# ethz-asl/multipoint

Hardware: AMD Instinct MI355X
Metric: image-pairs/sec (detect+desc+match) @ 480x640 (higher is better)
Workload: dtype f32

## Files before the change

multipoint_amd/csrc/forward.hip:

```cpp
#include "host.h"

using namespace mp_host;

namespace {

int pick_mbw(int H, int W)
{
    long long best = -1;
    int arg = 32;
    for (int mbw : {32, 16, 8}) {
        const int tw = mbw, th = 256 / mbw;
        const long long area = (long long)((H + th - 1) / th) * th * ((W + tw - 1) / tw) * tw;
        if (best < 0 || area < best) { best = area; arg = mbw; }
    }
    return arg;
}

void prof_begin(mp_handle* h, const char* name, double flop, hipStream_t s)
{
    if (!h->prof) return;
    if (h->prof_used == h->prof_entries.size()) {
        ProfEntry e{};
        (void)hipEventCreate(&e.a); (void)hipEventCreate(&e.b);
        h->prof_entries.push_back(e);
// ... 215 lines not shown
    w.Lg = w.Q + px * 16 * el;
    w.X = w.Lg + npx * (f16 ? 128 : 80) * el;
    w.R = w.X + npx * 128 * el;
    w.lists = w.R + (f16 ? npx * 256 * el : 0);
    w.bytes = w.lists + 2 * 1024 * 4 + 256;
    return w;
}

struct ImageRoute {
    int counts[2] = {0, 0};
    std::vector<int> ids;
};

ImageRoute route_images(const mp_handle* h, const unsigned char* is_optical, int B)
{
    ImageRoute r;
    if (!h->cfg.multispectral) { r.counts[0] = B; return r; }
    r.ids.assign(1024, 0);
    for (int b = 0; b < B; ++b) {
        if (is_optical[b]) r.ids[512 + r.counts[1]++] = b;
        else r.ids[r.counts[0]++] = b;
    }
    return r;
}

template <typename T>
int run_forward(mp_handle* h, const float* images, const ImageRoute& route, int B, int H, int W, float* prob, float* logits, float* desc,
                hipStream_t s)
{
    constexpr bool f16 = std::is_same<T, _Float16>::value;
    const FwdWorkspace w = fwd_workspace(f16, B, H, W);
    int rc;
    if ((rc = ensure(h, h->fwd_ws, w.bytes))) return rc;
    if (f16 && (rc = ensure(h, h->f16_dummy, 4096))) return rc;
    char* ws = static_cast<char*>(h->fwd_ws.p);
    T *P = reinterpret_cast<T*>(ws + w.P), *Q = reinterpret_cast<T*>(ws + w.Q), *X = reinterpret_cast<T*>(ws + w.X);
    T *Lg = reinterpret_cast<T*>(ws + w.Lg), *R = reinterpret_cast<T*>(ws + w.R);
    int* lists = reinterpret_cast<int*>(ws + w.lists);
    if (h->prof_used > 4000) h->prof_used = 0;

    if (h->cfg.multispectral)
        MP_HIP(hipMemcpyAsync(lists, route.ids.data(), 1024 * 4, hipMemcpyHostToDevice, s));
    for (int e = 0; e < 2; ++e) {
        const int nb = route.counts[e];
        if (nb == 0) continue;
        const Encoder& E = h->enc[e];
        const int* list = h->cfg.multispectral ? lists + 512 * e : nullptr;
        const EncoderPlan plan = plan_encoder(h, E, nb, B, H, W);
        if (!plan.conv[0].fuse_first) run_first(h, E, plan.conv[0].in_planar == MP_LAYOUT_PLANAR, images, P, nb, H, W, list, s);
        int hh = E.first_pool ? H / 2 : H, ww = E.first_pool ? W / 2 : W;
        T* src = P;
        T* dst = Q;
        for (int i = 0; i < E.nconv; ++i) {
            const ConvLayer& L = E.conv[i];
            if ((rc = run_conv(h, L, plan.conv[i], src, L.cin, 0, i == E.nconv - 1 ? X : dst, L.cout, 0, nb, hh, ww, list, s,
                               &E.first, images))) return rc;
            if (L.pool) { hh /= 2; ww /= 2; }
            T* t = src; src = dst; dst = t;
        }
    }

    const int Hc = H / 8, Wc = W / 8, lstride = f16 ? 128 : 80;
    const long long npx = (long long)B * Hc * Wc;
    const int D = h->cfg.descriptor_size;
    const int hc = h->head_channels;
    const int headc = h->cfg.descriptor_head ? 2 * hc : hc;
    const int encc = h->heads3.cin;
    ConvLaunch c3, c1x1;
    if constexpr (f16) {
        c3.kernel = f16_kind(h, h->heads3, encc, 0, false);
        c1x1.kernel = Kernel::f16;
    } else {
        c3.kernel = wino43_kind(h, h->heads3, Hc, Wc, encc, 0, headc, 0);
        plan_split_vin(h, h->heads3, B, Hc, Wc, B, c3);
    }
    if ((rc = run_conv(h, h->heads3, c3, X, encc, 0, P, headc, 0, B, Hc, Wc, nullptr, s))) return rc;
    if (h->dbg.head_fuse && (!f16 || prob || logits || desc)) {
        typename std::conditional<f16, HeadTailParamsH, HeadTailParams>::type t{};
        t.x = P; t.xstride = headc; t.K = hc;
        if constexpr (f16) {
            t.wdet = h->det1.wpack_h; t.bdet = h->det1.bias_h; t.wdesc = h->desc1.wpack_h; t.bdesc = h->desc1.bias_h;
        } else {
            t.wdet = h->det1.wpack; t.bdet = h->det1.bias; t.wdesc = h->desc1.wpack; t.bdesc = h->desc1.bias;
        }
        t.sdet = h->det1.scale; t.tdet = h->det1.shift; t.sdesc = h->desc1.scale; t.tdesc = h->desc1.shift;
        t.D = D; t.npx = npx; t.B = B; t.Hc = Hc; t.Wc = Wc;
        t.prob = prob; t.logits_nchw = logits; t.desc = desc;
        t.softmax_mode = h->cfg.softmax_mode; t.normalize = h->cfg.normalize_descriptors ? 1 : 0; t.ncu = h->ncu;
        prof_begin(h, "heads.tail", 2.0 * hc * (65.0 + (desc ? D : 0)) * (double)npx, s);
        int miss;
        if constexpr (f16) miss = launch_head_tail_f16(t, s); else miss = launch_head_tail(t, s);
        prof_end(h, s);
        if (!miss) return launch_status(h);
        if (h->prof) --h->prof_used;
        if (!h->head_fallback_noted) {
            h->head_fallback_noted = true;
            fprintf(stderr, "[multipoint_hip] note: fused head tail not instantiated for %d head channels / descriptor size %d: "
                            "using the separate 1x1 convolution, softmax and normalisation launches\n", hc, D);
        }
    }
    if ((rc = run_conv(h, h->det1, c1x1, P, headc, 0, Lg, lstride, 0, B, Hc, Wc, nullptr, s))) return rc;
    if (prob || logits) {
        prof_begin(h, "det.softmax_shuffle", 0.0, s);
        if constexpr (f16) launch_det_post_f16(Lg, lstride, B, Hc, Wc, prob, logits, h->cfg.softmax_mode, s);
        else launch_det_post(Lg, lstride, B, Hc, Wc, prob, logits, h->cfg.softmax_mode, s);
        prof_end(h, s);
    }
    if (desc) {
        T* raw;
        if constexpr (f16) raw = R; else raw = desc;
        if ((rc = run_conv(h, h->desc1, c1x1, P, headc, hc, raw, D, 0, B, Hc, Wc, nullptr, s))) return rc;
        prof_begin(h, "desc.l2norm", 0.0, s);
        if constexpr (f16) launch_desc_l2norm_f16(R, desc, npx, D, h->cfg.normalize_descriptors ? 1 : 0, s);
        else if (h->cfg.normalize_descriptors) launch_desc_l2norm(desc, desc, npx, D, 1, s);
        prof_end(h, s);
    }
    return launch_status(h);
}


struct BsWorkspace { size_t A, Bf, X, G, part, ss, lists, bytes; };
BsWorkspace bs_workspace(int B, int H, int W, bool multispectral)
{
    const size_t px = (size_t)B * H * W, npx = px / 64;
    BsWorkspace w{};
    w.Bf = w.A + px * 64 * 4;
    w.X = w.Bf + px * 64 * 4;
    w.G = w.X + npx * 128 * 4;
    w.part = w.G + (multispectral ? px * 4 : 0);
    w.ss = w.part + (size_t)MP_BN_MAX_PARTS * 2 * 512 * 8;
    w.lists = w.ss + 1024 * 4;
    w.bytes = w.lists + 2 * 1024 * 4 + 256;
    return w;
}

struct BsContext {
    mp_handle* h;
    double* part;
    float *scale, *shift;
    float* stats;
    hipStream_t s;
};

void bs_stats(BsContext& c, const float* x, long long npx, int C)
{
    prof_begin(c.h, "bn.stats", 0.0, c.s);
    launch_bn_stats(x, npx, C, C, c.part, c.s);
    prof_end(c.h, c.s);
}

void bs_finalize(BsContext& c, const float* x, long long npx, int C, int c0, int nc, int layer)
{
    const BnLayer& L = c.h->bn_layers[layer];
    prof_begin(c.h, "bn.finalize", 0.0, c.s);
    launch_bn_finalize(c.part, npx, C, x, c0, nc, L.channels, L.gamma, L.beta, c.scale, c.shift,
                       c.stats ? c.stats + L.offset : nullptr, c.stats ? c.stats + L.offset + L.channels : nullptr, c.s);
    prof_end(c.h, c.s);
}

void bs_apply(BsContext& c, const float* x, float* y, int B, int H, int W, int C, bool relu, bool pool, const int* out_list)
{
    prof_begin(c.h, "bn.apply", 0.0, c.s);
    launch_bn_apply(x, y, B, H, W, C, c.scale, c.shift, relu, pool, out_list, c.s);
    prof_end(c.h, c.s);
}

// ... 190 lines not shown
```

multipoint_amd/csrc/head_tail.hip:

```cpp
#include "mp_common.h"
#include "mp_device.h"

#include <type_traits>

namespace {

__device__ __forceinline__ float acc_rd(float a)
{
    float x;
    asm volatile("v_accvgpr_read_b32 %0, %1" : "=v"(x) : "a"(a));
    return x;
}
template <int ND>
__global__ __launch_bounds__(256) void head_tail_kernel(const HeadTailParams p)
{
    constexpr int NT = 3 + ND;
    constexpr int NP = 96 + 32 * ND;
    constexpr int WCH = 4 * NT * 256;
    constexpr int XCH = 2 * 4 * 256;
    __shared__ __attribute__((aligned(16))) float wl[2 * WCH];
    __shared__ __attribute__((aligned(16))) float xl[2 * 4 * XCH];
    __shared__ __attribute__((aligned(16))) float prm[3 * NP];
    const int tid = threadIdx.x, lane = tid & 63;
    const int wave = __builtin_amdgcn_readfirstlane(tid >> 6);
    const int pl = lane & 31, hf = lane >> 5;
    for (int i = tid; i < NP; i += 256) {
        const bool det = i < 96;
        const int c = det ? i : i - 96;
        prm[i] = det ? p.bdet[c] : p.bdesc[c];
        prm[NP + i] = det ? p.sdet[c] : p.sdesc[c];
        prm[2 * NP + i] = det ? p.tdet[c] : p.tdesc[c];
    }

    const long long ntiles = (p.npx + 127) / 128;
    long long tile = blockIdx.x;
    long long px = 0;
    bool valid = false;
    unsigned xoff = 0, xoff_next = 0;
    const float *xbase = p.x, *xbase_next = p.x;
    auto place = [&](long long t, unsigned& off, const float*& base) __attribute__((always_inline)) {
        const long long q = (t * 4 + wave) * 32 + pl;
        off = (unsigned)(((q < p.npx ? q : p.npx - 1) - t * 128) * p.xstride + hf * 4) * 4u;
        base = p.x + t * 128 * p.xstride;
    };
    place(tile, xoff, xbase);
    const int nchunks = p.K >> 5;
    const unsigned wl_lds = (unsigned)(size_t)wl, xl_lds = (unsigned)(size_t)xl + (unsigned)wave * (XCH * 4u);

    auto chunk_dma = [&](int c, int buf, int j, bool next_tile) __attribute__((always_inline)) {
        if (j < NT) {
            const int nb = j < 3 ? j : j - 3;
            const float* w = j < 3 ? p.wdet : p.wdesc;
            const float* src = w + (((((long long)(nb >> 1) * nchunks + c) * 4 + wave) * 2 + (nb & 1)) * 64) * 4;
            lds_dma<4, 0, 0>(src, (unsigned)lane * 16u, wl_lds + (unsigned)(buf * WCH + (wave * NT + j) * 256) * 4u);
        } else {
            const int q = j - NT, part = q >> 2, g = q & 3;
            if (ND == 0 && part == 1) return;
            lds_dma<4, 0, 0>((next_tile ? xbase_next : xbase) + part * p.K + c * 32 + g * 8, next_tile ? xoff_next : xoff,
                             xl_lds + (unsigned)(buf * 4 * XCH + (part * 4 + g) * 256) * 4u);
        }
    };

#pragma unroll
    for (int j = 0; j < NT + 8; ++j) chunk_dma(0, 0, j, false);
    dma_wait();
    __syncthreads();

    for (;;) {
    const bool has_next = tile + gridDim.x < ntiles;
    if (has_next) place(tile + gridDim.x, xoff_next, xbase_next);
    px = (tile * 4 + wave) * 32 + pl;
    valid = px < p.npx;
    f32x16 acc[NT];
#pragma unroll
    for (int t = 0; t < NT; ++t)
#pragma unroll
        for (int r = 0; r < 16; ++r) acc[t][r] = 0.f;

    auto chunk = [&](int c, auto buf_tag, bool prefetch, bool next_tile) __attribute__((always_inline)) {
        constexpr int buf = decltype(buf_tag)::value;
        const float* const wb = wl + buf * WCH + lane * 4;
        const float* const xb = xl + wave * XCH + buf * 4 * XCH + lane * 4;
        f32x4 wf[2][NT], xd[2], xs[2];
        auto frags = [&](int slot, int g) __attribute__((always_inline)) {
#pragma unroll
            for (int t = 0; t < NT; ++t) wf[slot][t] = *reinterpret_cast<const f32x4*>(&wb[(g * NT + t) * 256]);
            xd[slot] = *reinterpret_cast<const f32x4*>(&xb[g * 256]);
            if (ND) xs[slot] = *reinterpret_cast<const f32x4*>(&xb[(4 + g) * 256]);
        };
        frags(0, 0);
#pragma unroll
        for (int g = 0; g < 4; ++g) {
            if (g + 1 < 4) frags((g + 1) & 1, g + 1);
#pragma unroll
            for (int e = 0; e < 4; ++e)
#pragma unroll
                for (int t = 0; t < NT; ++t) {
                    acc[t] = __builtin_amdgcn_mfma_f32_32x32x2f32(wf[g & 1][t][e], t < 3 ? xd[g & 1][e] : xs[g & 1][e], acc[t], 0, 0, 0);
                    __builtin_amdgcn_sched_barrier(0);
                    const int m = (g * 4 + e) * NT + t;
                    if (prefetch && m < NT + 8) chunk_dma(next_tile ? 0 : c + 1, buf ^ 1, m, next_tile);
                    __builtin_amdgcn_sched_barrier(0);
                }
        }
        dma_wait();
        __syncthreads();
    };
    using B0 = std::integral_constant<int, 0>;
    using B1 = std::integral_constant<int, 1>;
    for (int c = 0; c < nchunks; c += 2) {
        chunk(c, B0{}, true, false);
        const bool lastc = c + 2 >= nchunks;
        chunk(c + 1, B1{}, !lastc || has_next, lastc);
    }

    const int cell = (int)(px % ((long long)p.Hc * p.Wc));
    const int b = (int)(px / ((long long)p.Hc * p.Wc));
    const int hc = cell / p.Wc, wc = cell - hc * p.Wc;
    {
        float v[32];
#pragma unroll
        for (int t = 0; t < 2; ++t)
#pragma unroll
            for (int r = 0; r < 16; ++r) {
                const int c = 32 * t + (r & 3) + 8 * (r >> 2) + 4 * hf;
                v[16 * t + r] = (acc_rd(acc[t][r]) + prm[c]) * prm[NP + c] + prm[2 * NP + c];
            }
        float d = (acc_rd(acc[2][0]) + prm[64]) * prm[NP + 64] + prm[2 * NP + 64];
        d = __shfl(d, pl);
        if (p.logits_nchw && valid) {
            const long long plane = (long long)p.Hc * p.Wc;
            float* o = p.logits_nchw + (long long)b * 65 * plane + cell;
#pragma unroll
            for (int t = 0; t < 2; ++t)
#pragma unroll
                for (int r = 0; r < 16; ++r) o[(long long)(32 * t + (r & 3) + 8 * (r >> 2) + 4 * hf) * plane] = v[16 * t + r];
            if (hf == 0) o[64 * plane] = d;
        }
        if (p.prob) {
            float m = 0.f;
            if (p.softmax_mode == 0) {
                m = d;
#pragma unroll
                for (int i = 0; i < 32; ++i) m = fmaxf(m, v[i]);
                m = fmaxf(m, __shfl_xor(m, 32));
            }
            float s = 0.f;
#pragma unroll
            for (int i = 0; i < 32; ++i) { v[i] = __expf(v[i] - m); s += v[i]; }
            s += __shfl_xor(s, 32);
            s += __expf(d - m);
            if (p.softmax_mode == 1) s += 0.00001f;
            const float rs = 1.0f / s;
            if (valid) {
                const int H = p.Hc * 8, W = p.Wc * 8;
                float* o = p.prob + ((long long)b * H + hc * 8) * W + wc * 8 + 4 * hf;
#pragma unroll
                for (int t = 0; t < 2; ++t)
#pragma unroll
                    for (int q = 0; q < 4; ++q) {
                        const f32x4 o4 = {v[16 * t + 4 * q] * rs, v[16 * t + 4 * q + 1] * rs, v[16 * t + 4 * q + 2] * rs,
                                          v[16 * t + 4 * q + 3] * rs};
                        *reinterpret_cast<f32x4*>(o + (long long)(4 * t + q) * W) = o4;
                    }
            }
        }
    }
    if constexpr (ND > 0) {
        if (p.desc) {
            float ss = 0.f;
            f32x4 dv[ND * 4];
#pragma unroll
            for (int t = 0; t < ND; ++t)
#pragma unroll
                for (int q = 0; q < 4; ++q)
#pragma unroll
                    for (int e = 0; e < 4; ++e) {
                        const int c = 32 * t + 8 * q + 4 * hf + e;
                        const float x = (acc_rd(acc[3 + t][4 * q + e]) + prm[96 + c]) * prm[NP + 96 + c] + prm[2 * NP + 96 + c];
                        dv[4 * t + q][e] = x;
                        ss += x * x;
                    }
            if (p.normalize) {
                ss += __shfl_xor(ss, 32);
                const float rd = 1.0f / fmaxf(sqrtf(ss), 1e-12f);
#pragma unroll
                for (int i = 0; i < ND * 4; ++i) dv[i] = dv[i] * rd;
            }
            if (valid) {
                float* o = p.desc + px * (32 * ND) + 4 * hf;
#pragma unroll
                for (int t = 0; t < ND; ++t)
#pragma unroll
                    for (int q = 0; q < 4; ++q) *reinterpret_cast<f32x4*>(o + 32 * t + 8 * q) = dv[4 * t + q];
            }
        }
    }
    if (!has_next) return;
    tile += gridDim.x;
    xoff = xoff_next; xbase = xbase_next;
    }
}

}

int launch_head_tail(const HeadTailParams& p, hipStream_t s)
{
    if (p.K % 64 != 0 || p.npx <= 0) return 1;
    const int D = p.desc ? p.D : 0;
    const long long tiles = (p.npx + 127) / 128;
    const dim3 grid((unsigned)(tiles < p.ncu ? tiles : p.ncu)), block(256);
    switch (D) {
    case 0: hipLaunchKernelGGL(head_tail_kernel<0>, grid, block, 0, s, p); return 0;
    case 64: hipLaunchKernelGGL(head_tail_kernel<2>, grid, block, 0, s, p); return 0;
    case 128: hipLaunchKernelGGL(head_tail_kernel<4>, grid, block, 0, s, p); return 0;
    case 256: hipLaunchKernelGGL(head_tail_kernel<8>, grid, block, 0, s, p); return 0;
    default: return 1;
    }
}
```

multipoint_amd/csrc/host.h:

```cpp
#pragma once
#include "../../include/multipoint_hip.h"
#include "mp_common.h"

#include <cmath>
#include <cstdio>
#include <cstdlib>
#include <cstring>
#include <string>
#include <type_traits>
#include <vector>

namespace mp_host {

inline std::string g_create_error;

struct DevBuf {
    void* p = nullptr;
    size_t bytes = 0;
    DevBuf(void* p_ = nullptr, size_t bytes_ = 0) : p(p_), bytes(bytes_) {}
    DevBuf(DevBuf&& o) noexcept : p(o.p), bytes(o.bytes) { o.p = nullptr; o.bytes = 0; }
    ~DevBuf() { if (p) (void)hipFree(p); }
};

struct ConvLayer {
    const char* name = "";
    float *wpack = nullptr, *bias = nullptr, *scale = nullptr, *shift = nullptr;
    float* u43pack = nullptr;
    float *u43pack_f1 = nullptr, *bias_f1 = nullptr;
    _Float16* wpack_h = nullptr;
    float* bias_h = nullptr;
    int cin = 0, cout = 0, taps = 9, nslices = 0;
    bool pool = false, relu = true;
};

struct FirstLayer {
    int channels = 64;
    float *w = nullptr, *bias = nullptr, *scale = nullptr, *shift = nullptr;
    float *w_h = nullptr, *bias_h = nullptr;
    float *w_f1 = nullptr, *bias_f1 = nullptr;
};

struct Encoder {
    FirstLayer first;
    ConvLayer conv[7];
    int nconv = 7;
    bool first_pool = false;
};

struct BnLayer {
    std::string name;
    int channels = 0;
    float *gamma = nullptr, *beta = nullptr;
    long long offset = 0;
};

struct ProfEntry {
    const char* name;
    hipEvent_t a, b;
    double flop;
};

struct DebugSwitches {
    bool winograd = true, wino43 = true, fuse_first = true, fuse43 = true, head_fuse = true, vin = true, planar = true;
    bool xplanar = true, f16_res = true, f16_fuse1 = true;
    int wino43_gen = 0, persist = 8, splitk_max = 8, f16_res_groups = 3;
};

struct ConvPolicy {
    bool direct = false;
    bool wino43 = true;
    int wino43_gen = 0;
    int splitk_max = 8;
};

}

struct mp_handle {
    mp_handle(int device_, int ncu_, int xcd_shift_, const mp_host::DebugSwitches& dbg_)
        : device(device_), ncu(ncu_), xcd_shift(xcd_shift_), dbg(dbg_) {}
    const int device;
    const int ncu, xcd_shift;
    const mp_host::DebugSwitches dbg;
    std::string err;
    bool loaded = false;
    mp_model_config cfg{};
    mp_host::ConvPolicy policy;
    std::vector<mp_host::DevBuf> weights;
    mp_host::Encoder enc[2];
    mp_host::ConvLayer heads3, det1, desc1;
    mp_host::DevBuf fwd_ws;
    mp_host::DevBuf nms_ws;
    mp_host::DevBuf match_ws;
    mp_host::DevBuf metrics_ws;
    mp_host::DevBuf split_ws;
    mp_host::DevBuf vin_ws;
    mp_host::DevBuf bs_ws;
    std::vector<mp_host::BnLayer> bn_layers;
    float* bn_ident = nullptr;
    mp_host::DevBuf nms_state;
    mp_host::DevBuf kp_scratch;
    mp_host::DevBuf nms_total;
    int last_nms_rounds = 0;
    mp_host::DevBuf tie_state;
    float tie_eps = 6e-5f;
    int tie_min = 4;
    int tie_last_B = 0;
    mp_host::DevBuf tie_pairs;
    int tie_pairs_min = 16;
    int head_channels = 256;
    mp_host::DevBuf f16_dummy;
    int* pinned = nullptr;
    bool prof = false;
    bool head_fallback_noted = false;
    std::vector<mp_host::ProfEntry> prof_entries;
    size_t prof_used = 0;
};

namespace mp_host {

inline int fail(mp_handle* h, int code, const std::string& msg)
{
    if (h) h->err = msg; else g_create_error = msg;
    return code;
}

#define MP_HIP(expr)                                                                          \
    do {                                                                                      \
        hipError_t _e = (expr);                                                               \
        if (_e != hipSuccess)                                                                 \
            return fail(h, MP_EHIP, std::string(#expr) + ": " + hipGetErrorString(_e));       \
    } while (0)

inline int ensure(mp_handle* h, DevBuf& b, size_t bytes)
{
    if (b.bytes >= bytes) return MP_OK;
    if (b.p) { MP_HIP(hipFree(b.p)); b.p = nullptr; b.bytes = 0; }
    hipError_t e = hipMalloc(&b.p, bytes);
    if (e != hipSuccess) {
        b.p = nullptr;
        return fail(h, MP_ENOMEM, "hipMalloc(" + std::to_string(bytes) + " B): " + hipGetErrorString(e));
    }
    b.bytes = bytes;
    return MP_OK;
}

inline int ensure_zeroed(mp_handle* h, DevBuf& b, size_t bytes, hipStream_t s)
{
    if (b.bytes >= bytes) return MP_OK;
    const int rc = ensure(h, b, bytes);
    if (rc == MP_OK) MP_HIP(hipMemsetAsync(b.p, 0, bytes, s));
    return rc;
}

inline int launch_status(mp_handle* h)
{
    MP_HIP(hipGetLastError());
    return MP_OK;
}

}
```

multipoint_amd/csrc/model_load.hip:

```cpp
#include "host.h"

#include <map>
#include <numeric>

using namespace mp_host;

namespace {

template <typename T, typename D>
int upload(mp_handle* h, const std::vector<T>& v, D** out)
{
    static_assert(sizeof(T) == sizeof(D), "upload: element size");
    void* d = nullptr;
    MP_HIP(hipMalloc(&d, v.size() * sizeof(T)));
    h->weights.emplace_back(d, v.size() * sizeof(T));
    MP_HIP(hipMemcpy(d, v.data(), v.size() * sizeof(T), hipMemcpyHostToDevice));
    *out = static_cast<D*>(d);
    return MP_OK;
}

void free_weights(mp_handle* h)
{
    h->weights.clear();
    h->bn_layers.clear();
    h->bn_ident = nullptr;
    h->loaded = false;
}

uint16_t f2h_bits(float f)
{
    uint32_t x;
    std::memcpy(&x, &f, 4);
    const uint32_t sign = (x >> 16) & 0x8000u;
    x &= 0x7fffffffu;
    if (x >= 0x7f800000u) return (uint16_t)(sign | 0x7c00u | (x > 0x7f800000u ? 0x200u : 0u));
    if (x >= 0x477ff000u) return (uint16_t)(sign | 0x7c00u);
    if (x < 0x38800000u) {
        if (x < 0x33000000u) return (uint16_t)sign;
        const int e = (int)(x >> 23);
        const uint32_t m = (x & 0x7fffffu) | 0x800000u;
        const int shift = 126 - e;
        uint32_t r = m >> shift;
        const uint32_t rem = m & ((1u << shift) - 1u), halfway = 1u << (shift - 1);
        if (rem > halfway || (rem == halfway && (r & 1u))) ++r;
        return (uint16_t)(sign | r);
    }
    uint32_t r = (((x >> 23) - 112u) << 10) | ((x & 0x7fffffu) >> 13);
    const uint32_t rem = x & 0x1fffu;
    if (rem > 0x1000u || (rem == 0x1000u && (r & 1u))) ++r;
    return (uint16_t)(sign | r);
}

float h2f_bits(uint16_t h)
{
    const uint32_t sign = (uint32_t)(h & 0x8000u) << 16;
    const uint32_t e = (h >> 10) & 0x1fu, m = h & 0x3ffu;
    uint32_t x;
    if (e == 0) {
        if (m == 0) { x = sign; }
        else {
            int sh = 0;
            uint32_t mm = m;
            while (!(mm & 0x400u)) { mm <<= 1; ++sh; }
            x = sign | ((uint32_t)(113 - sh) << 23) | ((mm & 0x3ffu) << 13);
        }
    } else if (e == 31) {
        x = sign | 0x7f800000u | (m << 13);
    } else {
        x = sign | ((e + 112u) << 23) | (m << 13);
    }
    float f;
    std::memcpy(&f, &x, 4);
    return f;
}

float round_half(float f) { return h2f_bits(f2h_bits(f)); }

struct TensorMap {
    std::map<std::string, const mp_tensor*> m;
    std::map<std::string, bool> used;
    const float* get(const std::string& k, long long numel, std::string& err)
    {
        auto it = m.find(k);
        if (it == m.end()) { err = "missing key in state_dict: " + k; return nullptr; }
        if (it->second->numel != numel) {
            err = "size mismatch for " + k + ": got " + std::to_string(it->second->numel) +
                  " elements, expected " + std::to_string(numel);
            return nullptr;
        }
        used[k] = true;
        return it->second->data;
    }
};

bool bn_terms(TensorMap& tm, const std::string& prefix, int c, int padded, std::vector<float>& scale,
              std::vector<float>& shift, std::string& err)
{
    const float* g = tm.get(prefix + ".weight", c, err); if (!g) return false;
    const float* b = tm.get(prefix + ".bias", c, err); if (!b) return false;
    const float* m = tm.get(prefix + ".running_mean", c, err); if (!m) return false;
    const float* v = tm.get(prefix + ".running_var", c, err); if (!v) return false;
    if (tm.m.count(prefix + ".num_batches_tracked")) tm.used[prefix + ".num_batches_tracked"] = true;
    scale.assign(padded, 1.f); shift.assign(padded, 0.f);
    for (int i = 0; i < c; ++i) {
        const float invstd = 1.0f / std::sqrt(v[i] + 1e-5f);
        const float alpha = invstd * g[i];
        scale[i] = alpha;
        shift[i] = b[i] - m[i] * alpha;
// ... 212 lines not shown
                    for (int k = 0; k < 9; ++k) g += w2[((size_t)o * 64 + c) * 9 + k];
                    acc += g * t1[c];
                }
            b2f[o] = (float)acc;
        }
        std::vector<float> u4;
        pack_wino43_weights({w2}, {64}, 64, 64, u4, own ? nullptr : s1.data());
        if ((rc = upload(h, wf, &E.first.w_f1))) return rc;
        if ((rc = upload(h, bf, &E.first.bias_f1))) return rc;
        if ((rc = upload(h, u4, &E.conv[0].u43pack_f1))) return rc;
        if ((rc = upload(h, b2f, &E.conv[0].bias_f1))) return rc;
    }
    return MP_OK;
}

ConvPolicy conv_policy(const DebugSwitches& d, const mp_model_config& cfg)
{
    ConvPolicy p;
    p.direct = cfg.conv_algorithm == 3 || (cfg.conv_algorithm == 0 && !d.winograd);
    p.wino43 = !p.direct && (cfg.conv_algorithm != 0 || d.wino43);
    p.wino43_gen = cfg.conv_algorithm == 1 ? 0 : cfg.conv_algorithm == 2 ? 2 : d.wino43_gen;
    p.splitk_max = cfg.batch_invariant ? 1 : d.splitk_max;
    return p;
}

}

extern "C" {

int mp_load_weights(mp_handle* h, const mp_model_config* cfg, const mp_tensor* tensors, int n_tensors)
{
    if (!h) return MP_EINVAL;
    if (!cfg || (!tensors && n_tensors > 0)) return fail(h, MP_EINVAL, "mp_load_weights: NULL argument");
    if (cfg->channel_version < 0 || cfg->channel_version > 2)
        return fail(h, MP_EINVAL, "unsupported model config: channel_version must be 0, 1 or 2 (MultiPoint.py:38-53)");
    if (cfg->channel_version != 0 && cfg->key_layout == 1)
        return fail(h, MP_EINVAL, "unsupported model config: SuperPointMagicLeap has channel_version 0 shapes");
    if (!cfg->double_convolution && cfg->key_layout == 1)
        return fail(h, MP_EINVAL, "unsupported model config: SuperPointMagicLeap has two convolutions per stage");
    if (cfg->descriptor_head && cfg->descriptor_size != 64 && cfg->descriptor_size != 128 &&
        cfg->descriptor_size != 256)
        return fail(h, MP_EINVAL, "unsupported model config: descriptor_size must be 64, 128 or 256");
    if (cfg->conv_algorithm < 0 || cfg->conv_algorithm > 3)
        return fail(h, MP_EINVAL, "unsupported model config: conv_algorithm must be 0 (auto), 1 (winograd43), 2 (winograd43_general) or 3 (direct)");
    MP_HIP(hipSetDevice(h->device));
    free_weights(h);
    h->cfg = *cfg;
    h->policy = conv_policy(h->dbg, *cfg);
    TensorMap tm;
    for (int i = 0; i < n_tensors; ++i) {
        if (!tensors[i].name || (!tensors[i].data && tensors[i].numel > 0))
            return fail(h, MP_EINVAL, "mp_load_weights: tensor " + std::to_string(i) + " has NULL field");
        tm.m[tensors[i].name] = &tensors[i];
    }
    int rc;
    if (cfg->key_layout == 1 && (cfg->multispectral || cfg->batchnorm || cfg->final_batchnorm))
        return fail(h, MP_EINVAL, "unsupported model config: SuperPointMagicLeap key layout has one encoder and no BatchNorm");
    if (!cfg->batchnorm && cfg->key_layout == 0)
        return fail(h, MP_EINVAL, "unsupported model config: MultiPoint key layout always has BatchNorm2d");
    if (cfg->multispectral) {
        if ((rc = build_encoder(h, tm, h->enc[0], "encoder_thermal"))) return rc;
        if ((rc = build_encoder(h, tm, h->enc[1], "encoder_optical"))) return rc;
    } else {
        if ((rc = build_encoder(h, tm, h->enc[0], "encoder"))) return rc;
    }
    const bool ml = cfg->key_layout == 1;
    const std::string det = "detector_head_convolutions", dsc = "descriptor_head_convolutions";
    const std::string bn3 = cfg->bn_first ? ".2" : ".3";
    const std::string det3 = ml ? "convPa" : det + ".1", dsc3 = ml ? "convDa" : dsc + ".1";
    const std::string det1k = ml ? "convPb" : det + ".4", dsc1k = ml ? "convDb" : dsc + ".4";
    const std::string det3bn = cfg->batchnorm ? det + bn3 : std::string(), dsc3bn = cfg->batchnorm ? dsc + bn3 : std::string();
    const std::string det1bn = cfg->final_batchnorm ? det + ".5" : std::string();
    const std::string dsc1bn = cfg->final_batchnorm ? dsc + ".5" : std::string();
    const int hc = cfg->channel_version == 0 ? 256 : cfg->descriptor_size;
    const int enc_out = h->enc[0].conv[h->enc[0].nconv - 1].cout;
    const int enc_real = cfg->channel_version == 2 ? 64 : 128;
    h->head_channels = hc;
    if (cfg->descriptor_head)
        rc = build_conv(h, tm, h->heads3, "heads.conv3x3", {det3, dsc3}, {det3bn, dsc3bn}, {hc, hc}, enc_out, 9, false, true, enc_real);
    else
        rc = build_conv(h, tm, h->heads3, "heads.conv3x3", {det3}, {det3bn}, {hc}, enc_out, 9, false, true, enc_real);
    if (rc) return rc;
    if ((rc = build_conv(h, tm, h->det1, "det.conv1x1", {det1k}, {det1bn}, {65}, hc, 1, false, false))) return rc;
    if (cfg->descriptor_head &&
        (rc = build_conv(h, tm, h->desc1, "desc.conv1x1", {dsc1k}, {dsc1bn}, {cfg->descriptor_size}, hc, 1, false, false)))
        return rc;
    if (cfg->batchnorm) {
        if ((rc = add_bn_layer(h, tm, det3bn, hc))) return rc;
        if (cfg->final_batchnorm && (rc = add_bn_layer(h, tm, det1bn, 65))) return rc;
        if (cfg->descriptor_head && (rc = add_bn_layer(h, tm, dsc3bn, hc))) return rc;
        if (cfg->descriptor_head && cfg->final_batchnorm && (rc = add_bn_layer(h, tm, dsc1bn, cfg->descriptor_size))) return rc;
        std::vector<float> ident(1024, 0.f);
        for (int i = 0; i < 512; ++i) ident[i] = 1.f;
        if ((rc = upload(h, ident, &h->bn_ident))) return rc;
    }
    for (auto& kv : tm.m)
        if (!tm.used.count(kv.first)) {
            if (kv.first.size() > 20 && kv.first.rfind(".num_batches_tracked") == kv.first.size() - 20) continue;
            free_weights(h);
            return fail(h, MP_EINVAL, "unexpected key in state_dict: " + kv.first);
        }
    h->loaded = true;
    return MP_OK;
}

}
```

multipoint_amd/csrc/mp_common.h:

```cpp
#pragma once
#include <hip/hip_runtime.h>
#include <stdint.h>

typedef float f32x16 __attribute__((ext_vector_type(16)));
typedef float f32x4 __attribute__((ext_vector_type(4)));

#define MP_WAVE 64

enum { MP_LAYOUT_NHWC = 0, MP_LAYOUT_PLANAR = 1, MP_LAYOUT_XPLANAR = 2 };

struct ConvParams {
    const float* in;
    float* out;
    const float* wpack;
    const float* bias;
    const float* scale;
    const float* shift;
    const int* img_list;
    const float* img;
    const float *w1, *b1, *s1, *t1;
    int B, H, W;
    int in_cstride, in_coff, cin;
    int out_cstride, out_coff, cout;
    int nslices;
// ... 81 lines not shown
    if (HI) asm("v_pk_fma_f32 %0, %1, %2, %3 op_sel:[0,1,0] op_sel_hi:[1,1,1] neg_lo:[1,0,0] neg_hi:[1,0,0]" : "=v"(d) : "v"(a), "s"(k), "v"(c));
    else asm("v_pk_fma_f32 %0, %1, %2, %3 op_sel:[0,0,0] op_sel_hi:[1,0,1] neg_lo:[1,0,0] neg_hi:[1,0,0]" : "=v"(d) : "v"(a), "s"(k), "v"(c));
    return d;
}
__device__ __forceinline__ void bt6(const mp_f32x2 d[6], mp_f32x2 r[6])
{
    const mp_f32x2 t0 = pk_fnma_k<1>(d[2], K_A2B2, d[4]);
    const mp_f32x2 t1 = pk_fnma_k<1>(d[1], K_A2B2, d[3]);
    const mp_f32x2 t2 = pk_fnma_k<0>(d[2], K_A2B2, d[4]);
    const mp_f32x2 t3 = pk_fnma_k<0>(d[1], K_A2B2, d[3]);
    r[0] = pk_fma_k<0>(d[0], K_PS, pk_fnma_k<1>(d[2], K_PS, d[4]));
    r[1] = pk_fma_k<0>(t1, K_AB, t0);
    r[2] = pk_fnma_k<0>(t1, K_AB, t0);
    r[3] = pk_fma_k<1>(t3, K_AB, t2);
    r[4] = pk_fnma_k<1>(t3, K_AB, t2);
    r[5] = pk_fma_k<0>(d[1], K_PS, pk_fnma_k<1>(d[3], K_PS, d[5]));
}
static_assert(MP_W43_B == 2 * MP_W43_A, "at6s() needs b = 2a");
__device__ __forceinline__ void at6s(const mp_f32x2 m[6], mp_f32x2 z[4])
{
    constexpr float a3 = (float)(MP_W43_A * MP_W43_A * MP_W43_A);
    const mp_f32x2 s1 = m[1] + m[2], d1 = m[1] - m[2], s2 = m[3] + m[4], d2 = m[3] - m[4];
    z[0] = (m[0] + s1) + s2;
    z[1] = __builtin_elementwise_fma(d2, mp_f32x2{2.f, 2.f}, d1);
    z[2] = __builtin_elementwise_fma(s2, mp_f32x2{4.f, 4.f}, s1);
    z[3] = __builtin_elementwise_fma(__builtin_elementwise_fma(d2, mp_f32x2{8.f, 8.f}, d1), mp_f32x2{a3, a3}, m[5]);
}
constexpr float w43_sigma(int r) { return r == 1 ? (float)MP_W43_A : r == 2 ? (float)(MP_W43_A * MP_W43_A) : 1.f; }
constexpr float w43_out_scale(int r, int c) { return w43_sigma(r) * w43_sigma(c); }
__device__ __forceinline__ mp_f32x2 w43_add_bias(mp_f32x2 z, int r, int c, mp_f32x2 bias)
{
    const float k = w43_out_scale(r, c);
    return k == 1.f ? z + bias : __builtin_elementwise_fma(z, mp_f32x2{k, k}, bias);
}
bool conv_wino43_supports(const ConvParams& p);
long long conv_wino43_items(const ConvParams& p);
long long conv_wino43_vglobal_floats(const ConvParams& p);
int launch_conv_wino43(const ConvParams& p, bool pool, hipStream_t s, bool fuse_first = false);
bool conv_wino43b_supports(const ConvParams& p);
int launch_conv_wino43b(const ConvParams& p, bool pool, hipStream_t s);
int launch_split_reduce(const ConvParams& p, int gen, bool pool, hipStream_t s);

struct ConvParamsH {
    const _Float16* in;
    _Float16* out;
    const _Float16* wpack;
    const float* bias;
    const float* scale;
    const float* shift;
    const int* img_list;
    int B, H, W;
    int in_cstride, in_coff, cin;
    int out_cstride, out_coff, cout;
    int nslices, tiles_x, tiles_y;
    int pad_zero, bn_first;
    long long total_px;
    unsigned magic_slices, magic_tx, magic_ty;
    int nitems;
    _Float16* dummy;
    int ncu, xcd_shift;
    int res_groups;
    const float* img;
    const float *w1, *b1, *s1, *t1;
};
struct Conv1ParamsH {
    const float* in;
    _Float16* out;
    const float* w;
    const float* bias; const float* scale; const float* shift;
    const int* img_list;
    int B, H, W;
    int pad_zero, bn_first;
    int pool;
};
int launch_conv_f16(const ConvParamsH& p, int taps, int mbw, bool pool, hipStream_t s);
bool conv_f16_res_supports(const ConvParamsH& p, int taps);
int launch_conv_f16_res(const ConvParamsH& p, int mbw, bool pool, hipStream_t s);
void launch_conv_first_f16(const Conv1ParamsH& p, hipStream_t s);

struct HeadTailParams {
    const float* x;
    int xstride, K;
    const float *wdet, *bdet, *sdet, *tdet;
    const float *wdesc, *bdesc, *sdesc, *tdesc;
    int D;
    long long npx;
    int B, Hc, Wc;
    float* prob;
    float* logits_nchw;
    float* desc;
    int softmax_mode;
    int normalize;
    int ncu;
};
int launch_head_tail(const HeadTailParams& p, hipStream_t s);
struct HeadTailParamsH {
    const _Float16* x;
    int xstride, K;
    const _Float16 *wdet, *wdesc;
    const float *bdet, *sdet, *tdet, *bdesc, *sdesc, *tdesc;
    int D;
    long long npx;
    int B, Hc, Wc;
    float* prob; float* logits_nchw; float* desc;
    int softmax_mode, normalize, ncu;
};
int launch_head_tail_f16(const HeadTailParamsH& p, hipStream_t s);
void launch_det_post(const float* logits, int lstride, int B, int Hc, int Wc, float* prob,
                     float* logits_nchw, int mode, hipStream_t s);
void launch_det_post_f16(const _Float16* logits, int lstride, int B, int Hc, int Wc, float* prob,
                         float* logits_nchw, int mode, hipStream_t s);
void launch_desc_l2norm(const float* raw, float* out, long long npx, int D, int normalize,
                        hipStream_t s);
void launch_desc_l2norm_f16(const _Float16* raw, float* out, long long npx, int D, int normalize,
                            hipStream_t s);

#define MP_NMS_MAX_R 15
struct NmsFootprint {
    int R;
    unsigned rowmask[2 * MP_NMS_MAX_R + 1];
};

void launch_nms_init(const float* prob, const uint8_t* mask, float min_prob, float* work,
                     long long n, hipStream_t s);
void launch_nms_round(float* work, int B, int H, int W, const NmsFootprint& fp, int* remaining,
                      int round, hipStream_t s, float tie_eps = 0.f, int* tie_pairs = nullptr);
void launch_nms_round0(const float* prob, const uint8_t* mask, float min_prob, float* work, int B, int H, int W,
                       const NmsFootprint& fp, int* remaining, hipStream_t s, int Ws, float tie_eps = 0.f, int* tie_pairs = nullptr);
void launch_nms_accumulate(int* remaining, int B, int H, int W, int round, int* total, hipStream_t s);
void launch_select_keypoints(const float* work, int B, int H, int W, int topk, int K,
                             int* list_idx, float* list_score, int list_cap, int* kp_yx,
                             float* kp_score, int* kp_count, float* prob_nms, int* seg_scratch, hipStream_t s,
                             float tie_eps = 0.f, int tie_min = 0, int* tie_state = nullptr, int Wout = 0,
                             int* tie_pairs = nullptr, int pairs_min = 0);
#define MP_TIE_MAX_IMAGES 1000
size_t keypoint_scratch_ints(int B, int H, int W);
void launch_extract_threshold(const float* map, const unsigned char* mask, int B, int H, int W, float thr, int K, int* kp_yx,
                              float* kp_score, int* kp_count, int* seg_scratch, hipStream_t s);

void launch_sample_desc(const float* desc, int B, int Hc, int Wc, int D, int H, int W,
                        const int* kp_yx, const int* kp_count, int K, float* out, hipStream_t s);

constexpr int MATCH_SHARES = 2;
void launch_match_impl(const float* dA, const int* nA, const float* dB, const int* nB,
                       long long pair_stride, int count_stride, int P, int K, int D, float thr,
                       unsigned long long* rowbest, unsigned long long* colbest, int* match_idx,
                       float* match_dist, int* match_count, hipStream_t s);

void launch_match_knn2(const float* dA, const int* nA, const float* dB, const int* nB, long long pair_stride,
                       int count_stride, int P, int K, int D, int* idx, float* dist, hipStream_t s);
void launch_match_threshold(const float* dA, const int* nA, const float* dB, const int* nB, long long pair_stride,
                            int count_stride, int P, int K, int D, float thr, int capacity, int* list_ij,
                            float* list_dist, int* list_count, hipStream_t s);

void launch_pair_metrics(const int* kp_yx, const int* kp_count, const int* match_idx, const double* hom, int P, int K,
                         int H, int W, float thr, double* warped, int* inv_idx, unsigned char* tp, int* metrics,
                         hipStream_t s);
void launch_repeatability(const int* kp_yx, const int* kp_count, const double* hom, int P, int K, int H, int W, double thr,
                          long long* warped, int* out, hipStream_t s);
void launch_ransac_homography(const int* kp_yx, const int* kp_count, const int* match_idx, int P, int K, int T, double thr,
                              unsigned long long seed, unsigned long long* best, double* H_out, unsigned char* mask,
                              int* n_inliers, hipStream_t s);

void launch_detector_metrics(const float* prob, const unsigned char* gt, int B, int H, int W, float zero_thr,
                             float distance_thr, unsigned long long* best, int* rec_index, float* rec_prob,
                             unsigned* rec_bits, int* rec_count, int* n_gt, hipStream_t s);
// ... 50 lines not shown
```

Before: 3461.

## Compute dustbin channel on CUDA cores and triple-buffer fused head tail

The fused detector/descriptor head tail no longer spends a whole 32-wide MFMA tile on the single 65th dustbin channel. That channel is now computed as a scalar FMA dot product from a separately uploaded weight row, interleaved with the MFMAs. The K loop is restructured into 16-wide chunks with a three-buffer LDS DMA pipeline and partial vmcnt waits, an XOR-swizzled activation layout, and two workgroups per CU for small descriptor sizes. This cuts MFMA work by a third for the detector part and deepens prefetch, at the cost of more LDS, a K<=256 restriction, and more barriers per pixel tile.

After: 3474 (median of 6 runs). Within noise of the previous version (+0.4%).

```diff
diff --git a/multipoint_amd/csrc/forward.hip b/multipoint_amd/csrc/forward.hip
--- a/multipoint_amd/csrc/forward.hip
+++ b/multipoint_amd/csrc/forward.hip
@@ -321,6 +321,7 @@
             t.wdet = h->det1.wpack_h; t.bdet = h->det1.bias_h; t.wdesc = h->desc1.wpack_h; t.bdesc = h->desc1.bias_h;
         } else {
             t.wdet = h->det1.wpack; t.bdet = h->det1.bias; t.wdesc = h->desc1.wpack; t.bdesc = h->desc1.bias;
+            t.wdust = h->det_dustbin;
         }
         t.sdet = h->det1.scale; t.tdet = h->det1.shift; t.sdesc = h->desc1.scale; t.tdesc = h->desc1.shift;
         t.D = D; t.npx = npx; t.B = B; t.Hc = Hc; t.Wc = Wc;
diff --git a/multipoint_amd/csrc/head_tail.hip b/multipoint_amd/csrc/head_tail.hip
--- a/multipoint_amd/csrc/head_tail.hip
+++ b/multipoint_amd/csrc/head_tail.hip
@@ -11,16 +11,22 @@
     asm volatile("v_accvgpr_read_b32 %0, %1" : "=v"(x) : "a"(a));
     return x;
 }
+template <int ND> constexpr int head_tail_wgs = ND <= 2 ? 2 : 1;
 template <int ND>
-__global__ __launch_bounds__(256) void head_tail_kernel(const HeadTailParams p)
+__global__ __launch_bounds__(256, head_tail_wgs<ND>) void head_tail_kernel(const HeadTailParams p)
 {
-    constexpr int NT = 3 + ND;
+    constexpr int NT = 2 + ND;
     constexpr int NP = 96 + 32 * ND;
-    constexpr int WCH = 4 * NT * 256;
-    constexpr int XCH = 2 * 4 * 256;
-    __shared__ __attribute__((aligned(16))) float wl[2 * WCH];
-    __shared__ __attribute__((aligned(16))) float xl[2 * 4 * XCH];
+    constexpr int WCH = 2 * NT * 256;
+    constexpr int XCH = (ND ? 2 : 1) * 2 * 256;
+    constexpr int NBUF = 3, PD = NBUF - 1;
+    constexpr int NWD = NT / 2, NXD = ND ? 4 : 2;
+    constexpr int NDMA = NWD + NXD;
+    static_assert(NT % 2 == 0, "a chunk's 2 * NT weight blocks are dealt evenly to the four waves");
+    __shared__ __attribute__((aligned(16))) float wl[NBUF * WCH];
+    __shared__ __attribute__((aligned(16))) float xl[NBUF * 4 * XCH];
     __shared__ __attribute__((aligned(16))) float prm[3 * NP];
+    __shared__ __attribute__((aligned(16))) float wdb[256];
     const int tid = threadIdx.x, lane = tid & 63;
     const int wave = __builtin_amdgcn_readfirstlane(tid >> 6);
     const int pl = lane & 31, hf = lane >> 5;
@@ -31,39 +37,49 @@
         prm[NP + i] = det ? p.sdet[c] : p.sdesc[c];
         prm[2 * NP + i] = det ? p.tdet[c] : p.tdesc[c];
     }
+    for (int i = tid; i < p.K; i += 256) wdb[i] = p.wdust[i];
 
     const long long ntiles = (p.npx + 127) / 128;
     long long tile = blockIdx.x;
     long long px = 0;
     bool valid = false;
-    unsigned xoff = 0, xoff_next = 0;
+    unsigned xoff[2] = {0, 0}, xoff_next[2] = {0, 0};
     const float *xbase = p.x, *xbase_next = p.x;
-    auto place = [&](long long t, unsigned& off, const float*& base) __attribute__((always_inline)) {
-        const long long q = (t * 4 + wave) * 32 + pl;
-        off = (unsigned)(((q < p.npx ? q : p.npx - 1) - t * 128) * p.xstride + hf * 4) * 4u;
+    auto place = [&](long long t, unsigned (&off)[2], const float*& base) __attribute__((always_inline)) {
+#pragma unroll
+        for (int h = 0; h < 2; ++h) {
+            const long long q = (t * 4 + wave) * 32 + 16 * h + (lane >> 2);
+            const int piece = (lane & 3) ^ ((lane >> 3) & 3);
+            off[h] = (unsigned)(((q < p.npx ? q : p.npx - 1) - t * 128) * p.xstride + piece * 4) * 4u;
+        }
         base = p.x + t * 128 * p.xstride;
     };
     place(tile, xoff, xbase);
-    const int nchunks = p.K >> 5;
+    const int nchunks = p.K >> 4;
     const unsigned wl_lds = (unsigned)(size_t)wl, xl_lds = (unsigned)(size_t)xl + (unsigned)wave * (XCH * 4u);
 
     auto chunk_dma = [&](int c, int buf, int j, bool next_tile) __attribute__((always_inline)) {
-        if (j < NT) {
-            const int nb = j < 3 ? j : j - 3;
-            const float* w = j < 3 ? p.wdet : p.wdesc;
-            const float* src = w + (((((long long)(nb >> 1) * nchunks + c) * 4 + wave) * 2 + (nb & 1)) * 64) * 4;
-            lds_dma<4, 0, 0>(src, (unsigned)lane * 16u, wl_lds + (unsigned)(buf * WCH + (wave * NT + j) * 256) * 4u);
+        if (j < NWD) {
+            const int kg = wave & 1, t = 2 * j + (wave >> 1);
+            const int nb = j == 0 ? t : t - 2;
+            const float* w = j == 0 ? p.wdet : p.wdesc;
+            const float* src = w + (((((long long)(nb >> 1) * (nchunks >> 1) + (c >> 1)) * 4 + (c & 1) * 2 + kg) * 2 + (nb & 1)) * 64) * 4;
+            lds_dma<4, 0, 0>(src, (unsigned)lane * 16u, wl_lds + (unsigned)(buf * WCH + (kg * NT + t) * 256) * 4u);
         } else {
-            const int q = j - NT, part = q >> 2, g = q & 3;
-            if (ND == 0 && part == 1) return;
-            lds_dma<4, 0, 0>((next_tile ? xbase_next : xbase) + part * p.K + c * 32 + g * 8, next_tile ? xoff_next : xoff,
-                             xl_lds + (unsigned)(buf * 4 * XCH + (part * 4 + g) * 256) * 4u);
+            const int q = j - NWD, part = q >> 1, h = q & 1;
+            lds_dma<4, 0, 0>((next_tile ? xbase_next : xbase) + part * p.K + c * 16, next_tile ? xoff_next[h] : xoff[h],
+                             xl_lds + (unsigned)(buf * 4 * XCH + (part * 2 + h) * 256) * 4u);
         }
     };
 
-#pragma unroll
-    for (int j = 0; j < NT + 8; ++j) chunk_dma(0, 0, j, false);
-    dma_wait();
+    int bufi = 0;
+    const int swz = (pl >> 1) & 3, xpix = (pl >> 4) * 256 + (pl & 15) * 16;
+#pragma unroll
+    for (int d = 0; d < PD; ++d) {
+#pragma unroll
+        for (int j = 0; j < NDMA; ++j) chunk_dma(d, d, j, false);
+    }
+    if (PD == 2) asm volatile("s_waitcnt vmcnt(%0)" :: "n"(NDMA) : "memory"); else dma_wait();
     __syncthreads();
 
     for (;;) {
@@ -72,46 +88,52 @@
     px = (tile * 4 + wave) * 32 + pl;
     valid = px < p.npx;
     f32x16 acc[NT];
+    float dust = 0.f;
 #pragma unroll
     for (int t = 0; t < NT; ++t)
 #pragma unroll
         for (int r = 0; r < 16; ++r) acc[t][r] = 0.f;
 
-    auto chunk = [&](int c, auto buf_tag, bool prefetch, bool next_tile) __attribute__((always_inline)) {
-        constexpr int buf = decltype(buf_tag)::value;
-        const float* const wb = wl + buf * WCH + lane * 4;
-        const float* const xb = xl + wave * XCH + buf * 4 * XCH + lane * 4;
-        f32x4 wf[2][NT], xd[2], xs[2];
+    for (int c = 0; c < nchunks; ++c) {
+        const int ct = c + PD;
+        const bool next_tile = ct >= nchunks;
+        const bool prefetch = !next_tile || has_next;
+        const int cf = next_tile ? ct - nchunks : ct;
+        int bt = bufi + PD; bt = bt >= NBUF ? bt - NBUF : bt;
+        const float* const wb = wl + bufi * WCH + lane * 4;
+        const float* const xb = xl + wave * XCH + bufi * 4 * XCH + xpix;
+        const float* const wd = wdb + c * 16;
+        f32x4 wf[2][NT], xd[2], xs[2], x0[2], x1[2], w0[2], w1[2];
         auto frags = [&](int slot, int g) __attribute__((always_inline)) {
 #pragma unroll
             for (int t = 0; t < NT; ++t) wf[slot][t] = *reinterpret_cast<const f32x4*>(&wb[(g * NT + t) * 256]);
-            xd[slot] = *reinterpret_cast<const f32x4*>(&xb[g * 256]);
-            if (ND) xs[slot] = *reinterpret_cast<const f32x4*>(&xb[(4 + g) * 256]);
+            xd[slot] = *reinterpret_cast<const f32x4*>(&xb[((2 * g + hf) ^ swz) * 4]);
+            if (ND) xs[slot] = *reinterpret_cast<const f32x4*>(&xb[512 + ((2 * g + hf) ^ swz) * 4]);
+            x0[slot] = *reinterpret_cast<const f32x4*>(&xb[((2 * g) ^ swz) * 4]);
+            x1[slot] = *reinterpret_cast<const f32x4*>(&xb[((2 * g + 1) ^ swz) * 4]);
+            w0[slot] = *reinterpret_cast<const f32x4*>(&wd[g * 8]);
+            w1[slot] = *reinterpret_cast<const f32x4*>(&wd[g * 8 + 4]);
         };
         frags(0, 0);
 #pragma unroll
-        for (int g = 0; g < 4; ++g) {
-            if (g + 1 < 4) frags((g + 1) & 1, g + 1);
+        for (int g = 0; g < 2; ++g) {
+            if (g == 0) frags(1, 1);
 #pragma unroll
             for (int e = 0; e < 4; ++e)
 #pragma unroll
                 for (int t = 0; t < NT; ++t) {
-                    acc[t] = __builtin_amdgcn_mfma_f32_32x32x2f32(wf[g & 1][t][e], t < 3 ? xd[g & 1][e] : xs[g & 1][e], acc[t], 0, 0, 0);
+                    acc[t] = __builtin_amdgcn_mfma_f32_32x32x2f32(wf[g][t][e], t < 2 ? xd[g][e] : xs[g][e], acc[t], 0, 0, 0);
+                    if (t == 0) dust = __builtin_fmaf(w0[g][e], x0[g][e], dust);
+                    if (t == 1) dust = __builtin_fmaf(w1[g][e], x1[g][e], dust);
                     __builtin_amdgcn_sched_barrier(0);
                     const int m = (g * 4 + e) * NT + t;
-                    if (prefetch && m < NT + 8) chunk_dma(next_tile ? 0 : c + 1, buf ^ 1, m, next_tile);
+                    if (m < NDMA) { if (prefetch) chunk_dma(cf, bt, m, next_tile); }
                     __builtin_amdgcn_sched_barrier(0);
                 }
         }
-        dma_wait();
+        if (PD == 2 && prefetch) asm volatile("s_waitcnt vmcnt(%0)" :: "n"(NDMA) : "memory"); else dma_wait();
         __syncthreads();
-    };
-    using B0 = std::integral_constant<int, 0>;
-    using B1 = std::integral_constant<int, 1>;
-    for (int c = 0; c < nchunks; c += 2) {
-        chunk(c, B0{}, true, false);
-        const bool lastc = c + 2 >= nchunks;
-        chunk(c + 1, B1{}, !lastc || has_next, lastc);
+        bufi = bufi + 1 == NBUF ? 0 : bufi + 1;
     }
 
     const int cell = (int)(px % ((long long)p.Hc * p.Wc));
@@ -126,8 +148,7 @@
                 const int c = 32 * t + (r & 3) + 8 * (r >> 2) + 4 * hf;
                 v[16 * t + r] = (acc_rd(acc[t][r]) + prm[c]) * prm[NP + c] + prm[2 * NP + c];
             }
-        float d = (acc_rd(acc[2][0]) + prm[64]) * prm[NP + 64] + prm[2 * NP + 64];
-        d = __shfl(d, pl);
+        const float d = (dust + prm[64]) * prm[NP + 64] + prm[2 * NP + 64];
         if (p.logits_nchw && valid) {
             const long long plane = (long long)p.Hc * p.Wc;
             float* o = p.logits_nchw + (long long)b * 65 * plane + cell;
@@ -177,7 +198,7 @@
 #pragma unroll
                     for (int e = 0; e < 4; ++e) {
                         const int c = 32 * t + 8 * q + 4 * hf + e;
-                        const float x = (acc_rd(acc[3 + t][4 * q + e]) + prm[96 + c]) * prm[NP + 96 + c] + prm[2 * NP + 96 + c];
+                        const float x = (acc_rd(acc[2 + t][4 * q + e]) + prm[96 + c]) * prm[NP + 96 + c] + prm[2 * NP + 96 + c];
                         dv[4 * t + q][e] = x;
                         ss += x * x;
                     }
@@ -198,7 +219,7 @@
     }
     if (!has_next) return;
     tile += gridDim.x;
-    xoff = xoff_next; xbase = xbase_next;
+    xoff[0] = xoff_next[0]; xoff[1] = xoff_next[1]; xbase = xbase_next;
     }
 }
 
@@ -206,15 +227,20 @@
 
 int launch_head_tail(const HeadTailParams& p, hipStream_t s)
 {
-    if (p.K % 64 != 0 || p.npx <= 0) return 1;
+    if (p.K % 64 != 0 || p.K > 256 || p.npx <= 0) return 1;
     const int D = p.desc ? p.D : 0;
     const long long tiles = (p.npx + 127) / 128;
-    const dim3 grid((unsigned)(tiles < p.ncu ? tiles : p.ncu)), block(256);
+    auto launch = [&](auto nd) {
+        constexpr int ND = decltype(nd)::value;
+        const long long wgs = (long long)head_tail_wgs<ND> * p.ncu;
+        hipLaunchKernelGGL(head_tail_kernel<ND>, dim3((unsigned)(tiles < wgs ? tiles : wgs)), dim3(256), 0, s, p);
+        return 0;
+    };
     switch (D) {
-    case 0: hipLaunchKernelGGL(head_tail_kernel<0>, grid, block, 0, s, p); return 0;
-    case 64: hipLaunchKernelGGL(head_tail_kernel<2>, grid, block, 0, s, p); return 0;
-    case 128: hipLaunchKernelGGL(head_tail_kernel<4>, grid, block, 0, s, p); return 0;
-    case 256: hipLaunchKernelGGL(head_tail_kernel<8>, grid, block, 0, s, p); return 0;
+    case 0: return launch(std::integral_constant<int, 0>{});
+    case 64: return launch(std::integral_constant<int, 2>{});
+    case 128: return launch(std::integral_constant<int, 4>{});
+    case 256: return launch(std::integral_constant<int, 8>{});
     default: return 1;
     }
 }
diff --git a/multipoint_amd/csrc/host.h b/multipoint_amd/csrc/host.h
--- a/multipoint_amd/csrc/host.h
+++ b/multipoint_amd/csrc/host.h
@@ -97,6 +97,7 @@
     mp_host::DevBuf bs_ws;
     std::vector<mp_host::BnLayer> bn_layers;
     float* bn_ident = nullptr;
+    float* det_dustbin = nullptr;
     mp_host::DevBuf nms_state;
     mp_host::DevBuf kp_scratch;
     mp_host::DevBuf nms_total;
diff --git a/multipoint_amd/csrc/model_load.hip b/multipoint_amd/csrc/model_load.hip
--- a/multipoint_amd/csrc/model_load.hip
+++ b/multipoint_amd/csrc/model_load.hip
@@ -24,6 +24,7 @@
     h->weights.clear();
     h->bn_layers.clear();
     h->bn_ident = nullptr;
+    h->det_dustbin = nullptr;
     h->loaded = false;
 }
 
@@ -402,6 +403,12 @@
         rc = build_conv(h, tm, h->heads3, "heads.conv3x3", {det3}, {det3bn}, {hc}, enc_out, 9, false, true, enc_real);
     if (rc) return rc;
     if ((rc = build_conv(h, tm, h->det1, "det.conv1x1", {det1k}, {det1bn}, {65}, hc, 1, false, false))) return rc;
+    {
+        std::string err;
+        const float* w = tm.get(det1k + ".weight", 65LL * hc, err);
+        if (!w) return fail(h, MP_EINVAL, err);
+        if ((rc = upload(h, std::vector<float>(w + 64LL * hc, w + 65LL * hc), &h->det_dustbin))) return rc;
+    }
     if (cfg->descriptor_head &&
         (rc = build_conv(h, tm, h->desc1, "desc.conv1x1", {dsc1k}, {dsc1bn}, {cfg->descriptor_size}, hc, 1, false, false)))
         return rc;
diff --git a/multipoint_amd/csrc/mp_common.h b/multipoint_amd/csrc/mp_common.h
--- a/multipoint_amd/csrc/mp_common.h
+++ b/multipoint_amd/csrc/mp_common.h
@@ -187,6 +187,7 @@
     const float* x;
     int xstride, K;
     const float *wdet, *bdet, *sdet, *tdet;
+    const float* wdust;
     const float *wdesc, *bdesc, *sdesc, *tdesc;
     int D;
     long long npx;
```
